# espnet/espnet

Hardware: NVIDIA H100
Metric: utterances/sec (RTF) Conformer-large ASR inference at 1/2/4/8 H100 vs CPU ref (higher is better)
Workload: dtype f32

## Files before the change

### espnet_b200/csrc/capi.cu

```cuda
#include <stdlib.h>
#include <string.h>

#include "common.cuh"
#include "gemm.h"

#ifndef ESPB_PDL_DEFAULT
#define ESPB_PDL_DEFAULT 1
#endif

static thread_local char g_err[512] = "";

void espb_set_error(const char* msg) {
  strncpy(g_err, msg ? msg : "", sizeof(g_err) - 1);
  g_err[sizeof(g_err) - 1] = 0;
}

namespace espb {
bool pdl_enabled() {
  static int v = -1;
  if (v < 0) { const char* e = getenv("ESPB_PDL"); v = e ? (e[0] == '1') : ESPB_PDL_DEFAULT; }
  return v == 1;
}
}

extern "C" {

const char* espb_last_error(void) { return g_err; }
int espb_abi_version(void) { return 7; }

int espb_device_sm(int* major, int* minor) {
  int dev = 0;
  cudaDeviceProp prop;
  if (cudaGetDevice(&dev) != cudaSuccess || cudaGetDeviceProperties(&prop, dev) != cudaSuccess) {
    espb_set_error("no CUDA device");
    return ESPB_ERR_CUDA;
  }
  *major = prop.major; *minor = prop.minor;
  return ESPB_OK;
}

int espb_gemm_f32(const EspbGemmDesc* d, int use_tc, cudaStream_t stream) {
  if (!d) { espb_set_error("gemm: null descriptor"); return ESPB_ERR_ARG; }
  if (d->a_mode < 0 || d->a_mode > 3) { espb_set_error("gemm: a_mode must be 0..3"); return ESPB_ERR_ARG; }
  return use_tc ? espb_gemm_tc_launch(*d, stream, use_tc == 2 ? 2 : 1) : espb_gemm_simt_launch(*d, stream);
}

}
```

### espnet_b200/csrc/gemm.cu

```cuda
#include <cuda.h>
#include <limits.h>

#include <algorithm>
#include <cmath>
#include <stdio.h>
#include <stdlib.h>

#include "common.cuh"
#include "gemm.h"
#include "tc_common.cuh"

namespace {

using namespace espb::tc;

constexpr int BM = 128;
constexpr int BK = 32;
constexpr int A_TILE_BYTES = BM * 128;
constexpr int NUM_THREADS = 512;
constexpr int EPI_WARP0 = 9;
constexpr int EPI_THREADS = NUM_THREADS - EPI_WARP0 * 32;
constexpr int STAGING_BYTES = 32768;
constexpr int LAUNCH_REGS = (65536 / NUM_THREADS) & ~7;
constexpr int CONSUMER_REGS = 176;
// ... 77 lines not shown
  }
#pragma unroll
  for (int i = 0; i < 4; ++i) {
    if (col + i >= N) break;
    if (e.split_out) { const float h = espb::tf32_hi(t[i]); crow[col + i] = h; crow[e.c_plane + col + i] = espb::tf32_lo(t[i], h); }
    else crow[col + i] = t[i];
  }
}

template <int BN>
__device__ __forceinline__ uint32_t staging_off(int r, int c) {
  return (uint32_t)(r * BN + ((((c >> 2) ^ ((r & 3) << 1))) << 2) + (c & 3)) * 4u;
}

template <int BN>
__device__ __forceinline__ void stage_tile(uint32_t buf, const float (&d)[BN / 2], int r0, int c0) {
#pragma unroll
  for (int j = 0; j < BN / 8; ++j)
#pragma unroll
    for (int h = 0; h < 2; ++h)
      asm volatile("st.shared.v2.f32 [%0], {%1, %2};" ::"r"(buf + staging_off<BN>(r0 + 8 * h, c0 + 8 * j)), "f"(d[4 * j + 2 * h]),
                   "f"(d[4 * j + 2 * h + 1])
                   : "memory");
}

__device__ __forceinline__ float4 ld_shared_f4(uint32_t addr) {
  float4 v;
  asm volatile("ld.shared.v4.f32 {%0, %1, %2, %3}, [%4];" : "=f"(v.x), "=f"(v.y), "=f"(v.z), "=f"(v.w) : "r"(addr) : "memory");
  return v;
}

constexpr int EPI_U = 4;

template <int BN>
__device__ __forceinline__ void epilogue_warps(const EspbGemmDesc& p, long long ntiles, int tiles_m, int tiles_n, int band, uint32_t staging,
                                               uint32_t stg_full, uint32_t stg_empty) {
  constexpr int NBUF = STAGING_BYTES / (64 * BN * 4);
  constexpr int TPR = BN / 4, RPP = EPI_THREADS / TPR;
  const int et = threadIdx.x - EPI_WARP0 * 32;
  const int r_first = et / TPR, cc = 4 * (et % TPR);
  int it = 0;
  for (long long t = blockIdx.x; t < ntiles; t += gridDim.x, ++it) {
    const TilePos tp = tile_at<BN>(p, t, tiles_m, tiles_n, band);
    EpiArgs e;
    const long long coff = (long long)tp.by * p.sc_y + (long long)tp.bx * p.sc_x;
    const long long roff = (long long)tp.by * p.sr_y + (long long)tp.bx * p.sr_x;
    e.C = p.C + coff; e.c_plane = p.c_plane; e.ldc = p.ldc; e.split_out = p.split_out;
    e.bias = p.bias ? p.bias + (long long)tp.bx * p.sbias_x : nullptr; e.R = p.R ? p.R + roff : nullptr;
    e.ldr = p.ldr; e.alpha = p.alpha; e.act = p.act;
    const bool c_vec = ((p.ldc & 3) == 0) && ((coff & 3) == 0) && ((p.c_plane & 3) == 0) && ((reinterpret_cast<uintptr_t>(p.C) & 15) == 0);
    const bool r_vec = ((p.ldr & 3) == 0) && ((reinterpret_cast<uintptr_t>(e.R) & 15) == 0);
    const int col = tp.n0 + cc;
    const float4 bv = e.bias ? ldg_quad(e.bias, col, p.N, (reinterpret_cast<uintptr_t>(e.bias) & 15) == 0) : make_float4(0.f, 0.f, 0.f, 0.f);
    for (int g = 0; g < 2; ++g) {
      mbar_wait(stg_full + 8 * g, (uint32_t)it & 1);
      const uint32_t buf = staging + (NBUF == 1 ? 0 : g) * (64 * BN * 4);
      const int row_base = tp.m0 + 64 * g;
#pragma unroll 1
      for (int r0 = r_first; r0 < 64; r0 += EPI_U * RPP) {
        float4 rv[EPI_U];
#pragma unroll
        for (int u = 0; u < EPI_U; ++u) {
          const int r = r0 + u * RPP, row = row_base + r;
          rv[u] = (e.R && r < 64 && row < p.M) ? ld_quad(e.R + (long long)row * e.ldr, col, p.N, r_vec) : make_float4(0.f, 0.f, 0.f, 0.f);
        }
#pragma unroll
        for (int u = 0; u < EPI_U; ++u) {
          const int r = r0 + u * RPP, row = row_base + r;
          if (r >= 64 || row >= p.M) break;
          const float4 a = ld_shared_f4(buf + staging_off<BN>(r, cc));
          const float v[4] = {epi_apply(e, a.x, bv.x, rv[u].x), epi_apply(e, a.y, bv.y, rv[u].y), epi_apply(e, a.z, bv.z, rv[u].z),
                              epi_apply(e, a.w, bv.w, rv[u].w)};
          epi_store4(e, row, col, v, p.N, c_vec);
        }
      }
      mbar_arrive_local(stg_empty + 8 * (NBUF == 1 ? g ^ 1 : g));
    }
  }
}

template <int BN, int STAGES, bool PROMOTE>
__global__ void __launch_bounds__(NUM_THREADS, 1)
gemm_tf32x3_kernel(const __grid_constant__ CUtensorMap tmA, const __grid_constant__ CUtensorMap tmB, EspbGemmDesc p, int bxm, int bym, int axm, int aym,
                   int tiles_m, int tiles_n, int band) {
  constexpr int B_TILE_BYTES = BN * 128;
  constexpr int STAGE_BYTES = 2 * A_TILE_BYTES + 2 * B_TILE_BYTES;
  constexpr int NR = BN / 2;
  constexpr int NBUF = STAGING_BYTES / (64 * BN * 4);
  extern __shared__ uint8_t smem_raw[];
  const uint32_t smem_base = (smem_u32(smem_raw) + 1023u) & ~1023u;
  const uint32_t staging = smem_base + STAGES * STAGE_BYTES;
  const uint32_t full_bar = staging + STAGING_BYTES, empty_bar = full_bar + 8 * STAGES;
  const uint32_t stg_full = empty_bar + 8 * STAGES, stg_empty = stg_full + 16;

  const int warp = threadIdx.x >> 5, lane = threadIdx.x & 31;
  const int num_kb = (p.K + BK - 1) / BK;
  const long long ntiles = (long long)tiles_m * tiles_n * p.nbx * p.nby;

  if (threadIdx.x == 0) {
    for (int s = 0; s < STAGES; ++s) { mbar_init(full_bar + 8 * s, 1); mbar_init(empty_bar + 8 * s, 2); }
    for (int g = 0; g < 2; ++g) { mbar_init(stg_full + 8 * g, 128); mbar_init(stg_empty + 8 * g, EPI_THREADS); }
    asm volatile("fence.mbarrier_init.release.cluster;" ::: "memory");
    asm volatile("prefetch.tensormap [%0];" ::"l"(&tmA) : "memory");
    asm volatile("prefetch.tensormap [%0];" ::"l"(&tmB) : "memory");
  }
  __syncthreads();
  espb::pdl_trigger();
  espb::pdl_wait();

  if (warp >= 8) {
    asm volatile("setmaxnreg.dec.sync.aligned.u32 %0;" ::"n"(EPI_REGS));
    if (warp >= EPI_WARP0) {
      epilogue_warps<BN>(p, ntiles, tiles_m, tiles_n, band, staging, stg_full, stg_empty);
      return;
    }
    if (elect_one_sync()) {
      const int cblk = (p.a_mode != 0) ? p.cv_cin / BK : 0;
      const ConvGeom g = conv_geom(p.a_mode);
      int s = 0;
      uint32_t ph = 0;
      for (long long t = blockIdx.x; t < ntiles; t += gridDim.x) {
        const TilePos tp = tile_at<BN>(p, t, tiles_m, tiles_n, band);
        for (int kb = 0; kb < num_kb; ++kb) {
          mbar_wait(empty_bar + 8 * s, ph ^ 1);
          const uint32_t fb = full_bar + 8 * s;
          mbar_expect_tx(fb, STAGE_BYTES);
          const uint32_t sa = smem_base + s * STAGE_BYTES;
          if (p.a_mode == 0) {
            const int ko = (p.kob > 0) ? kb / p.kob : 0;
            const int ki = (p.kob > 0) ? kb % p.kob : kb;
            tma_load_5d(sa, &tmA, fb, ki * BK, tp.m0, tp.bx * axm + ko, tp.by * aym, 0);
            tma_load_5d(sa + A_TILE_BYTES, &tmA, fb, ki * BK, tp.m0, tp.bx * axm + ko, tp.by * aym, 1);
          } else {
            const int tap = kb / cblk, c0 = (kb % cblk) * BK;
            const int kt = tap / g.k, kf = tap - kt * g.k;
            const int par = (kt % g.s) * g.s + kf % g.s;
            tma_load_5d(sa, &tmA, fb, c0, tp.m0 + kt / g.s, tp.bx + kf / g.s, par, tp.by);
            tma_load_5d(sa + A_TILE_BYTES, &tmA, fb, c0, tp.m0 + kt / g.s, tp.bx + kf / g.s, g.s * g.s + par, tp.by);
          }
          tma_load_5d(sa + 2 * A_TILE_BYTES, &tmB, fb, kb * BK, tp.n0, tp.bx * bxm, tp.by * bym, 0);
          tma_load_5d(sa + 2 * A_TILE_BYTES + B_TILE_BYTES, &tmB, fb, kb * BK, tp.n0, tp.bx * bxm, tp.by * bym, 1);
          if (++s == STAGES) { s = 0; ph ^= 1; }
        }
      }
    }
    return;
  }

  asm volatile("setmaxnreg.inc.sync.aligned.u32 %0;" ::"n"(CONSUMER_REGS));
  const int wg = warp >> 2;
  const bool wg_leader = (threadIdx.x & 127) == 0;
  const int row_in_half = (warp & 3) * 16 + (lane >> 2), col_in_tile = 2 * (lane & 3);
  const uint32_t my_buf = staging + (NBUF == 1 ? 0 : wg) * (64 * BN * 4);
  const uint32_t stg_parity0 = (NBUF == 1 && wg == 1) ? 0u : 1u;
  int s = 0;
  uint32_t ph = 0;
  float acc[NR], part[NR];
  int it = 0;
  for (long long t = blockIdx.x; t < ntiles; t += gridDim.x, ++it) {
#pragma unroll
    for (int i = 0; i < NR; ++i) { acc[i] = 0.f; part[i] = 0.f; }
    for (int kb = 0; kb < num_kb; ++kb) {
      mbar_wait(full_bar + 8 * s, ph);
      const uint32_t sa = smem_base + s * STAGE_BYTES + wg * 64 * 128;
      const uint32_t sb = smem_base + s * STAGE_BYTES + 2 * A_TILE_BYTES;
      const bool fresh = PROMOTE ? (kb % CHUNK_KB == 0) : (kb == 0);
      fence_regs(part);
      wgmma_fence();
#pragma unroll
      for (int k = 0; k < BK / 8; ++k) {
        const uint64_t a_hi = gmma_desc(sa + k * 32), a_lo = gmma_desc(sa + A_TILE_BYTES + k * 32);
        const uint64_t b_hi = gmma_desc(sb + k * 32), b_lo = gmma_desc(sb + B_TILE_BYTES + k * 32);
        wgmma_tf32<BN>(part, a_lo, b_hi, (fresh && k == 0) ? 0u : 1u);
        wgmma_tf32<BN>(part, a_hi, b_lo, 1u);
        wgmma_tf32<BN>(part, a_hi, b_hi, 1u);
      }
      wgmma_commit();
      wgmma_wait<0>();
      fence_regs(part);
      if (wg_leader) mbar_arrive_local(empty_bar + 8 * s);
      if (PROMOTE && (kb % CHUNK_KB == CHUNK_KB - 1 || kb == num_kb - 1)) {
#pragma unroll
        for (int i = 0; i < NR; ++i) acc[i] += part[i];
      }
      if (++s == STAGES) { s = 0; ph ^= 1; }
    }
    mbar_wait(stg_empty + 8 * wg, ((uint32_t)it & 1) ^ stg_parity0);
    stage_tile<BN>(my_buf, PROMOTE ? acc : part, row_in_half, col_in_tile);
    mbar_arrive_local(stg_full + 8 * wg);
  }
}

constexpr int BAND_MAX_KB = 4;
constexpr int BAND_SMEM = 232448;
constexpr int BAND_THREADS = 384;

struct BandTile {
  int k;
  int seq;
  int t, nt;
  int m0, n0;
  int bx, by;
};

__device__ __forceinline__ void band_unit(const EspbGemmDesc& p, int nmb, int k, int seq, int bn, BandTile& w) {
  const long long nunits = (long long)nmb * p.nbx * p.nby;
  for (;; ++k) {
    const long long u = blockIdx.x + (long long)k * gridDim.x;
    if (u >= nunits) { w.k = -1; return; }
    const int mb = (int)(u % nmb), z = (int)(u / nmb);
    const int m0 = mb * BM, mlast = min(p.M, m0 + BM) - 1;
    const int lo = max(0, p.band_t - 1 - mlast), hi = min(p.N - 1, 2 * p.band_t - 2 - m0);
    if (hi < lo) continue;
    const int n_start = lo & ~7;
    w.k = k; w.seq = seq; w.t = 0; w.nt = (hi - n_start) / bn + 1; w.m0 = m0; w.n0 = n_start; w.bx = z % p.nbx; w.by = z / p.nbx;
    return;
  }
}
__device__ __forceinline__ void band_next(const EspbGemmDesc& p, int nmb, int bn, BandTile& w) {
  if (w.t + 1 < w.nt) { ++w.t; w.n0 += bn; return; }
  band_unit(p, nmb, w.k + 1, w.seq + 1, bn, w);
}
// ... 222 lines not shown
      else c[0] = t;
    }
  }
}

int make_map(CUtensorMap* map, const float* base, const long long dims[5], const long long strides_el[4], int box_rows) {
  return espb_make_tensor_map(map, base, dims, strides_el, BK, box_rows, 1);
}

int num_sms() {
  static int n = 0;
  if (n == 0) {
    int dev = 0;
    cudaGetDevice(&dev);
    cudaDeviceGetAttribute(&n, cudaDevAttrMultiProcessorCount, dev);
    if (n <= 0) n = 1;
  }
  return n;
}

constexpr long long GEMM_B_L2_BYTES = 24ll << 20;
constexpr long long GEMM_B_BAND_BYTES = 8ll << 20;

int column_band(const EspbGemmDesc& d, int bn, int tiles_m, int tiles_n) {
  const double a_bytes = 2.0 * tiles_m * BM * d.K * sizeof(float), tile_b = 2.0 * bn * d.K * sizeof(float), b_bytes = tiles_n * tile_b;
  if (b_bytes <= GEMM_B_L2_BYTES) return tiles_n;
  const int w = (int)std::max(1.0, std::floor(GEMM_B_BAND_BYTES / tile_b));
  if (w >= tiles_n) return tiles_n;
  const double waves_per_b = tiles_m / std::max(1.0, (double)num_sms() / tiles_n);
  const double whole = a_bytes + b_bytes * waves_per_b, banded = a_bytes * ((tiles_n + w - 1) / w) + b_bytes;
  return banded < whole ? w : tiles_n;
}

template <int BN, int STAGES, bool PROMOTE>
int launch_tc(const CUtensorMap& tmA, const CUtensorMap& tmB, const EspbGemmDesc& d, int bxm, int bym, int axm, int aym, cudaStream_t stream) {
  constexpr int smem = STAGES * (2 * A_TILE_BYTES + 2 * BN * 128) + STAGING_BYTES + 1024 + 16 * STAGES + 32;
  static_assert(smem <= 232448, "dynamic shared memory budget exceeded");
  static bool attr_set = false;
  if (!attr_set) {
    if (cudaFuncSetAttribute(gemm_tf32x3_kernel<BN, STAGES, PROMOTE>, cudaFuncAttributeMaxDynamicSharedMemorySize, smem) != cudaSuccess) {
      espb_set_error("cudaFuncSetAttribute(max dynamic smem) failed");
      return ESPB_ERR_CUDA;
    }
    attr_set = true;
  }
  const int tiles_m = (d.M + BM - 1) / BM, tiles_n = (d.N + BN - 1) / BN;
  const int band = column_band(d, BN, tiles_m, tiles_n);
  const long long tiles = (long long)tiles_m * tiles_n * d.nbx * d.nby;
  const int grid = (int)std::min(tiles, (long long)num_sms());
  if (espb::launch_pdl(gemm_tf32x3_kernel<BN, STAGES, PROMOTE>, dim3(grid), dim3(NUM_THREADS), smem, stream, tmA, tmB, d, bxm, bym, axm, aym, tiles_m,
                       tiles_n, band) != cudaSuccess) {
    espb_set_error(cudaGetErrorString(cudaGetLastError())); return ESPB_ERR_CUDA;
  }
  return ESPB_OK;
}

void window_span(const float* base, long long ld, long long sx, long long sy, const EspbGemmDesc& d, uintptr_t& lo, uintptr_t& hi) {
  long long a = 0, b = (long long)(d.M - 1) * ld + (d.N - 1);
  const long long ex = (long long)(d.nbx - 1) * sx, ey = (long long)(d.nby - 1) * sy;
  (ex < 0 ? a : b) += ex;
  (ey < 0 ? a : b) += ey;
  lo = reinterpret_cast<uintptr_t>(base + a);
  hi = reinterpret_cast<uintptr_t>(base + b) + sizeof(float) - 1;
}

bool residual_ok(const EspbGemmDesc& d) {
  if (!d.R) return true;
  if (d.R == d.C && d.ldr == d.ldc && d.sr_x == d.sc_x && d.sr_y == d.sc_y) return true;
  uintptr_t rlo, rhi, clo, chi;
  window_span(d.R, d.ldr, d.sr_x, d.sr_y, d, rlo, rhi);
  for (int plane = 0; plane < (d.split_out ? 2 : 1); ++plane) {
    window_span(d.C + plane * d.c_plane, d.ldc, d.sc_x, d.sc_y, d, clo, chi);
    if (rlo <= chi && clo <= rhi) return false;
  }
  return true;
}

template <int NKB, bool PROMOTE>
int launch_band(const CUtensorMap& tmA, const CUtensorMap& tmB, const EspbGemmDesc& d, int bxm, int bym, int axm, int aym, cudaStream_t stream) {
  constexpr int BN = band_bn<NKB>();
  static bool attr_set = false;
  if (!attr_set) {
    if (cudaFuncSetAttribute(relpos_band_kernel<NKB, PROMOTE>, cudaFuncAttributeMaxDynamicSharedMemorySize, BAND_SMEM) != cudaSuccess) {
      espb_set_error("cudaFuncSetAttribute(max dynamic smem) failed (band GEMM)");
// ... 79 lines not shown
    if (d.kob > 0) { k_inner = (long long)d.kob * BK; n_outer = (d.K + k_inner - 1) / k_inner; }
    axm = (d.sa_x != 0 && d.nbx > 1) ? 1 : 0;
    aym = (d.sa_y != 0 && d.nby > 1) ? 1 : 0;
    long long dims[5] = {k_inner, d.M, (axm ? d.nbx : 1) + n_outer - 1, aym ? d.nby : 1, 2};
    long long str[4] = {d.lda, d.sa_x, d.sa_y, d.a_plane};
    rc = make_map(&tmA, d.A, dims, str, BM);
  } else {
    const ConvGeom g = conv_geom(d.a_mode);
    if (d.cv_cin % BK != 0 || d.K != g.k * g.k * d.cv_cin) {
      espb_set_error("conv gemm: cin must be a multiple of 32 and K = k*k*cin");
      return ESPB_ERR_ARG;
    }
    const long long sub = (long long)d.cv_f1h * d.cv_t1h * d.cv_cin, nph = g.s * g.s;
    long long dims[5] = {d.cv_cin, d.cv_t1h, d.cv_f1h, 2 * nph, d.nby};
    long long str[4] = {d.cv_cin, (long long)d.cv_t1h * d.cv_cin, sub, 2 * nph * sub};
    rc = make_map(&tmA, d.A, dims, str, BM);
  }
  if (rc != ESPB_OK) return rc;
  const int bxm = d.sb_x != 0 ? 1 : 0, bym = d.sb_y != 0 ? 1 : 0;
  if (d.band_t > 0 && d.a_mode == 0 && d.K <= BAND_MAX_KB * BK && !d.bias && !d.R && d.act == espb::ACT_NONE && !d.split_out) {
    const int nkb = (d.K + BK - 1) / BK;
    long long dims[5] = {d.K, d.N, bxm ? d.nbx : 1, bym ? d.nby : 1, 2};
    long long str[4] = {d.ldb, d.sb_x, d.sb_y, d.b_plane};
    if ((rc = make_map(&tmB, d.B, dims, str, nkb <= 3 ? band_bn<3>() : band_bn<4>())) != ESPB_OK) return rc;
    const bool pr = version == 2;
    switch (nkb) {
      case 1: return pr ? launch_band<1, true>(tmA, tmB, d, bxm, bym, axm, aym, stream) : launch_band<1, false>(tmA, tmB, d, bxm, bym, axm, aym, stream);
      case 2: return pr ? launch_band<2, true>(tmA, tmB, d, bxm, bym, axm, aym, stream) : launch_band<2, false>(tmA, tmB, d, bxm, bym, axm, aym, stream);
      case 3: return pr ? launch_band<3, true>(tmA, tmB, d, bxm, bym, axm, aym, stream) : launch_band<3, false>(tmA, tmB, d, bxm, bym, axm, aym, stream);
      default: return pr ? launch_band<4, true>(tmA, tmB, d, bxm, bym, axm, aym, stream) : launch_band<4, false>(tmA, tmB, d, bxm, bym, axm, aym, stream);
    }
  }
  const long long tiles_m = (d.M + BM - 1) / BM, nb = (long long)d.nbx * d.nby;
  const int bn = (d.N <= 64 || tiles_m * ((d.N + 127) / 128) * nb < num_sms()) ? 64 : 128;
  {
    long long dims[5] = {d.K, d.N, bxm ? d.nbx : 1, bym ? d.nby : 1, 2};
    long long str[4] = {d.ldb, d.sb_x, d.sb_y, d.b_plane};
    rc = make_map(&tmB, d.B, dims, str, bn);
    if (rc != ESPB_OK) return rc;
  }
  if (version == 2) {
    if (bn == 128) return launch_tc<128, 3, true>(tmA, tmB, d, bxm, bym, axm, aym, stream);
    return launch_tc<64, 4, true>(tmA, tmB, d, bxm, bym, axm, aym, stream);
  }
  if (bn == 128) return launch_tc<128, 3, false>(tmA, tmB, d, bxm, bym, axm, aym, stream);
  return launch_tc<64, 4, false>(tmA, tmB, d, bxm, bym, axm, aym, stream);
}

int espb_gemm_simt_launch(const EspbGemmDesc& d, cudaStream_t stream) {
  if (d.M <= 0 || d.N <= 0 || d.K <= 0 || d.nbx <= 0 || d.nby <= 0) { espb_set_error("gemm: bad shape"); return ESPB_ERR_ARG; }
  if (!residual_ok(d)) { espb_set_error("gemm: residual R partially overlaps the output C"); return ESPB_ERR_ARG; }
  dim3 grid((d.M + 63) / 64, (d.N + 63) / 64, d.nbx * d.nby);
  gemm_simt_kernel<<<grid, 256, 0, stream>>>(d);
  ESPB_CHECK_LAUNCH();
  return ESPB_OK;
}
```

### espnet_b200/csrc/gemm.h

```cpp
#pragma once
#include <cuda_runtime.h>

struct EspbGemmDesc {
  int M, N, K;
  int nbx, nby;
  int a_mode;
  int kob;
  const float* A; long long a_plane, lda, sa_x, sa_y;
  const float* B; long long b_plane, ldb, sb_x, sb_y;
  float* C; long long c_plane, ldc, sc_x, sc_y;
  int split_out;
  const float* bias;
  long long sbias_x;
  const float* R; long long ldr, sr_x, sr_y;
  float alpha;
  int act;
  int cv_t1h, cv_f1h, cv_cin;
  int band_t;
};

struct ConvGeom { int k, s; };
__host__ __device__ __forceinline__ ConvGeom conv_geom(int a_mode) {
  return a_mode == 2 ? ConvGeom{3, 1} : a_mode == 3 ? ConvGeom{5, 3} : ConvGeom{3, 2};
}

int espb_gemm_tc_launch(const EspbGemmDesc& d, cudaStream_t stream, int version);
int espb_gemm_simt_launch(const EspbGemmDesc& d, cudaStream_t stream);
```

### espnet_b200/lib.py

```python
import ctypes
import os
from ctypes import POINTER, Structure, c_float, c_int, c_longlong, c_void_p

import torch

_HERE = os.path.dirname(os.path.abspath(__file__))
LIB_PATH = os.path.join(_HERE, "libespnet_b200.so")

_lib = None


class GemmDesc(Structure):

    _fields_ = [
        ("M", c_int), ("N", c_int), ("K", c_int), ("nbx", c_int), ("nby", c_int), ("a_mode", c_int), ("kob", c_int),
        ("A", c_void_p), ("a_plane", c_longlong), ("lda", c_longlong), ("sa_x", c_longlong), ("sa_y", c_longlong),
        ("B", c_void_p), ("b_plane", c_longlong), ("ldb", c_longlong), ("sb_x", c_longlong), ("sb_y", c_longlong),
        ("C", c_void_p), ("c_plane", c_longlong), ("ldc", c_longlong), ("sc_x", c_longlong), ("sc_y", c_longlong),
        ("split_out", c_int), ("bias", c_void_p), ("sbias_x", c_longlong),
        ("R", c_void_p), ("ldr", c_longlong), ("sr_x", c_longlong), ("sr_y", c_longlong),
        ("alpha", c_float), ("act", c_int), ("cv_t1h", c_int), ("cv_f1h", c_int), ("cv_cin", c_int), ("band_t", c_int),
    ]


P, I, L, F = c_void_p, c_int, c_longlong, c_float

_SIGS = {
    "espb_gemm_f32": [POINTER(GemmDesc), I, P],
    "espb_stft_logmel_f32": [P, P, I, I, I, P, P, P, P, P, P, P, I, I, P, I, P, P],
    "espb_utt_mvn_from_partial_f32": [P, P, I, I, I, I, P, P],
    "espb_utt_mvn_f32": [P, P, I, I, I, P, P],
    "espb_global_mvn_f32": [P, P, I, I, I, P, P, I, I, P],
    "espb_layernorm_f32": [P, L, I, P, P, F, P, P, L, P],
    "espb_split_tf32_f32": [P, L, P, L, P],
    "espb_conv1_relu_f32": [P, I, I, I, P, P, I, P, I, I, I, I, P],
    "espb_conv1_relu_phase_f32": [P, I, I, I, P, P, I, P, I, I, I, I, I, P],
    "espb_phase_split_f32": [P, L, I, I, I, I, I, I, I, P, P],
    "espb_qu_qv_f32": [P, L, L, I, P, P, P, P, L, P],
    "espb_v_transpose_f32": [P, L, I, I, I, I, P, P, L, I, P],
    "espb_relpos_softmax_f32": [P, P, I, I, I, I, I, P, F, P, L, P],
    "espb_masked_softmax_f32": [P, I, I, I, I, P, F, P, L, P],
    "espb_flash_attn_f32": [P, L, L, L, P, L, L, L, P, L, I, P, I, P, I, I, I, I, P, L, L, P],
    "espb_glu_dwconv_bn_swish_f32": [P, I, I, I, P, P, P, I, P, P, P, L, P],
    "espb_zero_pad_rows_f32": [P, I, I, I, P, L, I, P],
    "espb_csgu_f32": [P, I, I, I, P, P, P, F, P, P, I, P, P, L, P],
    "espb_merge_dwconv_f32": [P, I, I, I, P, P, P, I, P, L, P],
    "espb_branch_pool_f32": [P, P, L, I, I, I, P, P, P, P, P, P, P, P],
    "espb_branch_merge_f32": [P, P, L, L, I, I, P, F, F, P, L, P],
    "espb_cbe_build_chunks_f32": [P, I, I, I, I, I, I, P, I, I, F, P, P, P, P],
    "espb_cbe_ctx_propagate_f32": [P, I, I, I, I, P, P, I, I, P],
    "espb_zero_rows_f32": [P, L, L, L, I, L, I, P],
    "espb_gather_rows_f32": [P, I, L, P, I, I, P, P],
    "espb_log_softmax_rows_f32": [P, L, L, I, P],
    "espb_argmax_rows_f32": [P, L, L, I, P, P],
# ... 90 lines not shown
```

### espnet_b200/ops.py

```python
import os

import torch

from . import lib
from .lib import GemmDesc, call, ptr

ACT_NONE, ACT_RELU, ACT_SWISH, ACT_GELU = 0, 1, 2, 3

_GEMM_MODE = os.environ.get("ESPNET_B200_GEMM", "tc2")
launch_counter = [0]
gemm_profile = None


def set_gemm_mode(mode):
    global _GEMM_MODE
    assert mode in ("tc", "tc2", "simt")
    _GEMM_MODE = mode


def gemm_mode():
    return _GEMM_MODE


def _count(n=1):
    launch_counter[0] += n


def new_split(*shape, device="cuda"):
    return torch.empty((2,) + tuple(shape), dtype=torch.float32, device=device)


def split_from(x):
    x = x.contiguous()
    out = new_split(*x.shape, device=x.device)
    call("espb_split_tf32_f32", ptr(x), x.numel(), ptr(out), x.numel())
    _count()
    return out


def gemm(M, N, K, A, a_plane, lda, B, b_plane, ldb, C, ldc, *, c_plane=0, split_out=False, bias=None, R=None, ldr=0,
         alpha=1.0, act=ACT_NONE, nbx=1, nby=1, sa=(0, 0), sb=(0, 0), sc=(0, 0), sr=(0, 0), kob=0, a_mode=0, conv=(0, 0, 0),
         a_off=0, b_off=0, c_off=0, r_off=0, sbias_x=0, bias_off=0, band_t=0, force=None):
    d = GemmDesc()
    d.M, d.N, d.K, d.nbx, d.nby, d.a_mode, d.kob = M, N, K, nbx, nby, a_mode, kob
    d.A = A.data_ptr() + 4 * a_off
    d.a_plane, d.lda, d.sa_x, d.sa_y = a_plane, lda, sa[0], sa[1]
    d.B = B.data_ptr() + 4 * b_off
    d.b_plane, d.ldb, d.sb_x, d.sb_y = b_plane, ldb, sb[0], sb[1]
    d.C = C.data_ptr() + 4 * c_off
    d.c_plane, d.ldc, d.sc_x, d.sc_y = c_plane, ldc, sc[0], sc[1]
    d.split_out = 1 if split_out else 0
    d.bias = (bias.data_ptr() + 4 * bias_off) if bias is not None else None
    d.sbias_x = sbias_x
    d.R = (R.data_ptr() + 4 * r_off) if R is not None else None
    d.ldr, d.sr_x, d.sr_y = ldr, sr[0], sr[1]
    d.alpha, d.act = float(alpha), act
    d.cv_t1h, d.cv_f1h, d.cv_cin = conv
    d.band_t = band_t
    mode = force or _GEMM_MODE
    use_tc = {"tc": 1, "tc2": 2}.get(mode, 0)
    if use_tc:
        al = [lda, ldb, a_plane, b_plane, sa[0], sa[1], sb[0], sb[1], a_off, b_off]
        if any(v % 4 for v in al):
            use_tc = 0
        if a_mode and conv[2] % 32:
            use_tc = 0
        if a_mode == 0 and kob > 0 and K % (kob * 32):
            use_tc = 0
    if lib.profile is not None:
        lib.profile_tag[0] = f"{'tc' + str(use_tc) if use_tc else 'simt'} M{M} N{N} K{K} x{nbx * nby}" + (" conv" if a_mode else "")
    prof = gemm_profile if use_tc else None
    if prof is not None:
        e0, e1 = torch.cuda.Event(enable_timing=True), torch.cuda.Event(enable_timing=True)
        e0.record()
    call("espb_gemm_f32", d, use_tc)
    if prof is not None:
        e1.record()
        n_alg = band_t if band_t > 0 else N
        prof.append((2.0 * M * n_alg * K * nbx * nby, e0, e1))
    _count()
    return bool(use_tc)


def linear(x_split, w_split, out, *, bias=None, act=ACT_NONE, residual=None, alpha=1.0, split_out=False, force=None):
    M, K = x_split.shape[1], x_split.shape[2]
    N = w_split.shape[1]
    assert w_split.shape[2] == K
    return gemm(M, N, K, x_split, M * K, K, w_split, N * K, K, out, N, c_plane=M * N, split_out=split_out, bias=bias,
                R=residual, ldr=N, alpha=alpha, act=act, force=force)


_ATTN_MODE = os.environ.get("ESPB_ATTN", "fused")


def set_attn_mode(mode):
    global _ATTN_MODE
    assert mode in ("fused", "materialized")
    _ATTN_MODE = mode


def attn_mode():
    return _ATTN_MODE


def use_flash_attn(dk):
    return _ATTN_MODE == "fused" and dk == 64 and _GEMM_MODE != "simt"


def flash_attn(q_split, q_off, ldq, k_split, k_off, ldk, vt, Tp, bd, Rp, lens32, B, H, T, dk, out_split):
    call("espb_flash_attn_f32", ptr(q_split), q_off, q_split[0].numel(), ldq, ptr(k_split), k_off, k_split[0].numel(), ldk, ptr(vt),
         vt[0].numel(), Tp, ptr(bd), Rp, ptr(lens32), B, H, T, dk, ptr(out_split), out_split[0].numel(), H * dk)
    _count()


def layernorm(x, gamma, beta, eps, out_plain=None, out_split=None):
    rows, D = x.numel() // x.shape[-1], x.shape[-1]
    plane = out_split[0].numel() if out_split is not None else 0
    call("espb_layernorm_f32", ptr(x), rows, D, ptr(gamma), ptr(beta), eps, ptr(out_plain), ptr(out_split), plane)
    _count()


def log_softmax_rows_(x2d):
# ... 13 lines not shown
```

### include/espnet_b200.h

```cpp
#ifndef ESPNET_B200_H
#define ESPNET_B200_H

#include <cuda_runtime.h>

#ifdef __cplusplus
extern "C" {
#endif

#define ESPB_ACT_NONE 0
#define ESPB_ACT_RELU 1
#define ESPB_ACT_SWISH 2
#define ESPB_ACT_GELU 3

const char* espb_last_error(void);
int espb_abi_version(void);
int espb_device_sm(int* major, int* minor);

typedef struct EspbGemmDesc {
  int M, N, K;
  int nbx, nby;
  int a_mode;
  int kob;
  const float* A; long long a_plane, lda, sa_x, sa_y;
  const float* B; long long b_plane, ldb, sb_x, sb_y;
  float* C; long long c_plane, ldc, sc_x, sc_y;
  int split_out;
  const float* bias; long long sbias_x;
  const float* R; long long ldr, sr_x, sr_y;
  float alpha;
  int act;
  int cv_t1h, cv_f1h, cv_cin;
  int band_t;
} EspbGemmDesc;
int espb_gemm_f32(const EspbGemmDesc* d, int use_tc, cudaStream_t stream);

int espb_frontend_blocks(int Tf_max);
int espb_stft_logmel_f32(const float* wave, const long long* wave_lens, int B, int Lmax, int hop, const float* window, const float* tw512,
                         const float* tw256t, const int* mel_start, const int* mel_count, const int* mel_offset, const float* mel_weight,
                         int mel_nnz, int n_mels, float* out, int Tf_max, float* partial, cudaStream_t stream);
int espb_utt_mvn_from_partial_f32(float* feats, const long long* wave_lens, int B, int Tf_max, int n_mels, int hop, const float* partial,
                                  cudaStream_t stream);
int espb_utt_mvn_f32(float* feats, const long long* feat_lens, int B, int Tf_max, int n_mels, float* partial_ws, cudaStream_t stream);
int espb_global_mvn_f32(float* feats, const long long* feat_lens, int B, int Tmax, int D, const float* mean, const float* stdv, int norm_means,
                        int norm_vars, cudaStream_t stream);

int espb_layernorm_f32(const float* x, long long rows, int D, const float* gamma, const float* beta, float eps, float* out_plain,
                       float* out_split, long long split_plane, cudaStream_t stream);
int espb_split_tf32_f32(const float* x, long long n, float* out, long long plane, cudaStream_t stream);
int espb_conv1_relu_f32(const float* feats, int B, int Tf_max, int F, const float* w, const float* bias, int C, float* out, int T1, int F1,
                        int T1h, int F1h, cudaStream_t stream);
int espb_conv1_relu_phase_f32(const float* feats, int B, int Tf_max, int F, const float* w, const float* bias, int C, float* out, int T1, int F1,
                              int s, int T1h, int F1h, cudaStream_t stream);
int espb_phase_split_f32(const float* x, long long x_plane, int B, int F, int T, int C, int s, int Th, int Fh, float* out, cudaStream_t stream);
int espb_qu_qv_f32(const float* qkv, long long qkv_plane, long long M, int D, const float* pos_u, const float* pos_v, float* qu, float* qv,
                   long long out_plane, cudaStream_t stream);
int espb_v_transpose_f32(const float* qkv, long long qkv_plane, int B, int Tmax, int D, int H, const int* lens, float* vt,
                         long long vt_plane, int Tp, cudaStream_t stream);
int espb_relpos_softmax_f32(const float* ac, const float* bd, int B, int H, int T, int Tp, int Rp, const int* lens, float sqrt_dk,
                            float* probs, long long probs_plane, cudaStream_t stream);
int espb_masked_softmax_f32(const float* scores, int B, int H, int T, int Tp, const int* lens, float sqrt_dk, float* probs, long long probs_plane,
                            cudaStream_t stream);
int espb_flash_attn_f32(const float* q, long long q_off, long long q_plane, long long ldq, const float* k, long long k_off, long long k_plane,
                        long long ldk, const float* vt, long long vt_plane, int Tp, const float* bd, int Rp, const int* lens, int B, int H, int T,
                        int dk, float* out, long long out_plane, long long ldo, cudaStream_t stream);
int espb_glu_dwconv_bn_swish_f32(const float* y, int B, int Tmax, int C, const int* lens, const float* dw_w, const float* dw_b, int K,
// ... 68 lines not shown
```

Before: 182.4.

## Add split-K stream-K style path to TF32x3 TMA GEMM with workspace reduction

Adds optional split-K for the promoted TF32x3 tensor-core GEMM when a caller supplies a workspace. Each tile is divided into K-chunk units spread across CTAs. Non-leading splits stage partial chunk sums to global slots, and the last arriving unit reduces them with atomic tickets before applying the epilogue. A host cost model picks the split factor and BN to fill the SMs for small-tile-count GEMMs, at the price of extra global traffic and synchronisation.

```diff
diff --git a/espnet_b200/csrc/capi.cu b/espnet_b200/csrc/capi.cu
--- a/espnet_b200/csrc/capi.cu
+++ b/espnet_b200/csrc/capi.cu
@@ -42,6 +42,10 @@
 int espb_gemm_f32(const EspbGemmDesc* d, int use_tc, cudaStream_t stream) {
   if (!d) { espb_set_error("gemm: null descriptor"); return ESPB_ERR_ARG; }
   if (d->a_mode < 0 || d->a_mode > 3) { espb_set_error("gemm: a_mode must be 0..3"); return ESPB_ERR_ARG; }
+  if (d->ws && ((reinterpret_cast<uintptr_t>(d->ws) & 15) || d->ws_bytes < 0)) {
+    espb_set_error("gemm: split-K workspace must be 16-byte aligned with ws_bytes >= 0");
+    return ESPB_ERR_ARG;
+  }
   return use_tc ? espb_gemm_tc_launch(*d, stream, use_tc == 2 ? 2 : 1) : espb_gemm_simt_launch(*d, stream);
 }
 
diff --git a/espnet_b200/csrc/gemm.cu b/espnet_b200/csrc/gemm.cu
--- a/espnet_b200/csrc/gemm.cu
+++ b/espnet_b200/csrc/gemm.cu
@@ -133,6 +133,59 @@
 
 constexpr int EPI_U = 4;
 
+struct SplitK {
+  int S;
+  int cpu;
+  int nch;
+  int nslots;
+  float* part;
+  int* ctr;
+};
+
+__device__ __forceinline__ float4 ld_cg_f4(const float* ptr) {
+  float4 v;
+  asm volatile("ld.global.cg.v4.f32 {%0, %1, %2, %3}, [%4];" : "=f"(v.x), "=f"(v.y), "=f"(v.z), "=f"(v.w) : "l"(ptr) : "memory");
+  return v;
+}
+__device__ __forceinline__ void add_f4(float4& a, const float4& b) { a.x += b.x; a.y += b.y; a.z += b.z; a.w += b.w; }
+__device__ __forceinline__ void epi_bar_sync() { asm volatile("bar.sync 1, %0;" ::"n"(EPI_THREADS) : "memory"); }
+
+template <int BN>
+__device__ __forceinline__ void stage_to_slot(int rows, float* slot, uint32_t staging, uint32_t stg_full, uint32_t stg_empty, int it,
+                                              int r_first, int cc) {
+  constexpr int NBUF = STAGING_BYTES / (64 * BN * 4);
+  constexpr int RPP = EPI_THREADS / (BN / 4);
+  for (int g = 0; g < 2; ++g) {
+    mbar_wait(stg_full + 8 * g, (uint32_t)it & 1);
+    const uint32_t buf = staging + (NBUF == 1 ? 0 : g) * (64 * BN * 4);
+#pragma unroll 1
+    for (int r = r_first; r < min(64, rows - 64 * g); r += RPP)
+      *reinterpret_cast<float4*>(slot + (64 * g + r) * BN + cc) = ld_shared_f4(buf + staging_off<BN>(r, cc));
+    mbar_arrive_local(stg_empty + 8 * (NBUF == 1 ? g ^ 1 : g));
+  }
+}
+
+struct TileEpi {
+  EpiArgs e;
+  bool c_vec, r_vec;
+  int col;
+  float4 bv;
+};
+__device__ __forceinline__ TileEpi tile_epi(const EspbGemmDesc& p, const TilePos& tp, int cc) {
+  TileEpi te;
+  EpiArgs& e = te.e;
+  const long long coff = (long long)tp.by * p.sc_y + (long long)tp.bx * p.sc_x;
+  const long long roff = (long long)tp.by * p.sr_y + (long long)tp.bx * p.sr_x;
+  e.C = p.C + coff; e.c_plane = p.c_plane; e.ldc = p.ldc; e.split_out = p.split_out;
+  e.bias = p.bias ? p.bias + (long long)tp.bx * p.sbias_x : nullptr; e.R = p.R ? p.R + roff : nullptr;
+  e.ldr = p.ldr; e.alpha = p.alpha; e.act = p.act;
+  te.c_vec = ((p.ldc & 3) == 0) && ((coff & 3) == 0) && ((p.c_plane & 3) == 0) && ((reinterpret_cast<uintptr_t>(p.C) & 15) == 0);
+  te.r_vec = ((p.ldr & 3) == 0) && ((reinterpret_cast<uintptr_t>(e.R) & 15) == 0);
+  te.col = tp.n0 + cc;
+  te.bv = e.bias ? ldg_quad(e.bias, te.col, p.N, (reinterpret_cast<uintptr_t>(e.bias) & 15) == 0) : make_float4(0.f, 0.f, 0.f, 0.f);
+  return te;
+}
+
 template <int BN>
 __device__ __forceinline__ void epilogue_warps(const EspbGemmDesc& p, long long ntiles, int tiles_m, int tiles_n, int band, uint32_t staging,
                                                uint32_t stg_full, uint32_t stg_empty) {
@@ -143,16 +196,8 @@
   int it = 0;
   for (long long t = blockIdx.x; t < ntiles; t += gridDim.x, ++it) {
     const TilePos tp = tile_at<BN>(p, t, tiles_m, tiles_n, band);
-    EpiArgs e;
-    const long long coff = (long long)tp.by * p.sc_y + (long long)tp.bx * p.sc_x;
-    const long long roff = (long long)tp.by * p.sr_y + (long long)tp.bx * p.sr_x;
-    e.C = p.C + coff; e.c_plane = p.c_plane; e.ldc = p.ldc; e.split_out = p.split_out;
-    e.bias = p.bias ? p.bias + (long long)tp.bx * p.sbias_x : nullptr; e.R = p.R ? p.R + roff : nullptr;
-    e.ldr = p.ldr; e.alpha = p.alpha; e.act = p.act;
-    const bool c_vec = ((p.ldc & 3) == 0) && ((coff & 3) == 0) && ((p.c_plane & 3) == 0) && ((reinterpret_cast<uintptr_t>(p.C) & 15) == 0);
-    const bool r_vec = ((p.ldr & 3) == 0) && ((reinterpret_cast<uintptr_t>(e.R) & 15) == 0);
-    const int col = tp.n0 + cc;
-    const float4 bv = e.bias ? ldg_quad(e.bias, col, p.N, (reinterpret_cast<uintptr_t>(e.bias) & 15) == 0) : make_float4(0.f, 0.f, 0.f, 0.f);
+    const TileEpi te = tile_epi(p, tp, cc);
+    const EpiArgs& e = te.e;
     for (int g = 0; g < 2; ++g) {
       mbar_wait(stg_full + 8 * g, (uint32_t)it & 1);
       const uint32_t buf = staging + (NBUF == 1 ? 0 : g) * (64 * BN * 4);
@@ -163,16 +208,16 @@
 #pragma unroll
         for (int u = 0; u < EPI_U; ++u) {
           const int r = r0 + u * RPP, row = row_base + r;
-          rv[u] = (e.R && r < 64 && row < p.M) ? ld_quad(e.R + (long long)row * e.ldr, col, p.N, r_vec) : make_float4(0.f, 0.f, 0.f, 0.f);
+          rv[u] = (e.R && r < 64 && row < p.M) ? ld_quad(e.R + (long long)row * e.ldr, te.col, p.N, te.r_vec) : make_float4(0.f, 0.f, 0.f, 0.f);
         }
 #pragma unroll
         for (int u = 0; u < EPI_U; ++u) {
           const int r = r0 + u * RPP, row = row_base + r;
           if (r >= 64 || row >= p.M) break;
           const float4 a = ld_shared_f4(buf + staging_off<BN>(r, cc));
-          const float v[4] = {epi_apply(e, a.x, bv.x, rv[u].x), epi_apply(e, a.y, bv.y, rv[u].y), epi_apply(e, a.z, bv.z, rv[u].z),
-                              epi_apply(e, a.w, bv.w, rv[u].w)};
-          epi_store4(e, row, col, v, p.N, c_vec);
+          const float v[4] = {epi_apply(e, a.x, te.bv.x, rv[u].x), epi_apply(e, a.y, te.bv.y, rv[u].y), epi_apply(e, a.z, te.bv.z, rv[u].z),
+                              epi_apply(e, a.w, te.bv.w, rv[u].w)};
+          epi_store4(e, row, te.col, v, p.N, te.c_vec);
         }
       }
       mbar_arrive_local(stg_empty + 8 * (NBUF == 1 ? g ^ 1 : g));
@@ -180,10 +225,56 @@
   }
 }
 
+template <int BN>
+__device__ __forceinline__ void epilogue_split_warps(const EspbGemmDesc& p, long long ntiles, int tiles_m, int tiles_n, int band,
+                                                     uint32_t staging, uint32_t stg_full, uint32_t stg_empty, const SplitK& sk, int* ticket) {
+  constexpr int TPR = BN / 4, RPP = EPI_THREADS / TPR;
+  constexpr int SLOT = BM * BN;
+  const int et = threadIdx.x - EPI_WARP0 * 32;
+  const int r_first = et / TPR, cc = 4 * (et % TPR);
+  int it = 0;
+  const long long nunits = ntiles * sk.S;
+  for (long long u = blockIdx.x; u < nunits; u += gridDim.x) {
+    const long long t = u / sk.S;
+    const int sp = (int)(u - t * sk.S);
+    const TilePos tp = tile_at<BN>(p, t, tiles_m, tiles_n, band);
+    float* const tws = sk.part + t * sk.nslots * SLOT;
+    const int c0 = sp * sk.cpu, c1 = min(c0 + sk.cpu, sk.nch);
+    for (int c = sp == 0 ? c1 - 1 : c0; c < c1; ++c, ++it)
+      stage_to_slot<BN>(p.M - tp.m0, tws + (sp == 0 ? 0 : 1 + c - sk.cpu) * SLOT, staging, stg_full, stg_empty, it, r_first, cc);
+    __threadfence();
+    epi_bar_sync();
+    if (et == 0) *ticket = atomicAdd(sk.ctr + t, 1);
+    epi_bar_sync();
+    if (*reinterpret_cast<volatile int*>(ticket) != sk.S - 1) continue;
+    __threadfence();
+    const TileEpi te = tile_epi(p, tp, cc);
+    const EpiArgs& e = te.e;
+    for (int r = r_first; r < BM; r += RPP) {
+      const int row = tp.m0 + r;
+      if (row >= p.M) break;
+      const float* const src = tws + r * BN + cc;
+      const float4 rv = e.R ? ld_quad(e.R + (long long)row * e.ldr, te.col, p.N, te.r_vec) : make_float4(0.f, 0.f, 0.f, 0.f);
+      float4 a = ld_cg_f4(src);
+      int k = 1;
+      for (; k + 4 <= sk.nslots; k += 4) {
+        const float4 v0 = ld_cg_f4(src + k * SLOT), v1 = ld_cg_f4(src + (k + 1) * SLOT), v2 = ld_cg_f4(src + (k + 2) * SLOT),
+                     v3 = ld_cg_f4(src + (k + 3) * SLOT);
+        add_f4(a, v0); add_f4(a, v1); add_f4(a, v2); add_f4(a, v3);
+      }
+      for (; k < sk.nslots; ++k) add_f4(a, ld_cg_f4(src + k * SLOT));
+      const float v[4] = {epi_apply(e, a.x, te.bv.x, rv.x), epi_apply(e, a.y, te.bv.y, rv.y), epi_apply(e, a.z, te.bv.z, rv.z),
+                          epi_apply(e, a.w, te.bv.w, rv.w)};
+      epi_store4(e, row, te.col, v, p.N, te.c_vec);
+    }
+    if (et == 0) sk.ctr[t] = 0;
+  }
+}
+
 template <int BN, int STAGES, bool PROMOTE>
 __global__ void __launch_bounds__(NUM_THREADS, 1)
 gemm_tf32x3_kernel(const __grid_constant__ CUtensorMap tmA, const __grid_constant__ CUtensorMap tmB, EspbGemmDesc p, int bxm, int bym, int axm, int aym,
-                   int tiles_m, int tiles_n, int band) {
+                   int tiles_m, int tiles_n, int band, SplitK sk) {
   constexpr int B_TILE_BYTES = BN * 128;
   constexpr int STAGE_BYTES = 2 * A_TILE_BYTES + 2 * B_TILE_BYTES;
   constexpr int NR = BN / 2;
@@ -197,6 +288,9 @@
   const int warp = threadIdx.x >> 5, lane = threadIdx.x & 31;
   const int num_kb = (p.K + BK - 1) / BK;
   const long long ntiles = (long long)tiles_m * tiles_n * p.nbx * p.nby;
+  const long long nunits = ntiles * sk.S;
+  const int kb_split = sk.S > 1 ? sk.cpu * CHUNK_KB : num_kb;
+  __shared__ int split_ticket;
 
   if (threadIdx.x == 0) {
     for (int s = 0; s < STAGES; ++s) { mbar_init(full_bar + 8 * s, 1); mbar_init(empty_bar + 8 * s, 2); }
@@ -212,7 +306,8 @@
   if (warp >= 8) {
     asm volatile("setmaxnreg.dec.sync.aligned.u32 %0;" ::"n"(EPI_REGS));
     if (warp >= EPI_WARP0) {
-      epilogue_warps<BN>(p, ntiles, tiles_m, tiles_n, band, staging, stg_full, stg_empty);
+      if (PROMOTE && sk.S > 1) epilogue_split_warps<BN>(p, ntiles, tiles_m, tiles_n, band, staging, stg_full, stg_empty, sk, &split_ticket);
+      else epilogue_warps<BN>(p, ntiles, tiles_m, tiles_n, band, staging, stg_full, stg_empty);
       return;
     }
     if (elect_one_sync()) {
@@ -220,9 +315,11 @@
       const ConvGeom g = conv_geom(p.a_mode);
       int s = 0;
       uint32_t ph = 0;
-      for (long long t = blockIdx.x; t < ntiles; t += gridDim.x) {
+      for (long long u = blockIdx.x; u < nunits; u += gridDim.x) {
+        const long long t = u / sk.S;
         const TilePos tp = tile_at<BN>(p, t, tiles_m, tiles_n, band);
-        for (int kb = 0; kb < num_kb; ++kb) {
+        const int kb0 = (int)(u - t * sk.S) * kb_split, kb1 = min(kb0 + kb_split, num_kb);
+        for (int kb = kb0; kb < kb1; ++kb) {
           mbar_wait(empty_bar + 8 * s, ph ^ 1);
           const uint32_t fb = full_bar + 8 * s;
           mbar_expect_tx(fb, STAGE_BYTES);
@@ -258,10 +355,19 @@
   uint32_t ph = 0;
   float acc[NR], part[NR];
   int it = 0;
-  for (long long t = blockIdx.x; t < ntiles; t += gridDim.x, ++it) {
+  auto handover = [&](const float (&v)[NR]) {
+    mbar_wait(stg_empty + 8 * wg, ((uint32_t)it & 1) ^ stg_parity0);
+    stage_tile<BN>(my_buf, v, row_in_half, col_in_tile);
+    mbar_arrive_local(stg_full + 8 * wg);
+    ++it;
+  };
+  for (long long u = blockIdx.x; u < nunits; u += gridDim.x) {
+    const long long t = u / sk.S;
+    const int sp = (int)(u - t * sk.S);
+    const int kb0 = sp * kb_split, kb1 = min(kb0 + kb_split, num_kb);
 #pragma unroll
     for (int i = 0; i < NR; ++i) { acc[i] = 0.f; part[i] = 0.f; }
-    for (int kb = 0; kb < num_kb; ++kb) {
+    for (int kb = kb0; kb < kb1; ++kb) {
       mbar_wait(full_bar + 8 * s, ph);
       const uint32_t sa = smem_base + s * STAGE_BYTES + wg * 64 * 128;
       const uint32_t sb = smem_base + s * STAGE_BYTES + 2 * A_TILE_BYTES;
@@ -281,14 +387,16 @@
       fence_regs(part);
       if (wg_leader) mbar_arrive_local(empty_bar + 8 * s);
       if (PROMOTE && (kb % CHUNK_KB == CHUNK_KB - 1 || kb == num_kb - 1)) {
-#pragma unroll
-        for (int i = 0; i < NR; ++i) acc[i] += part[i];
+        if (sp == 0) {
+#pragma unroll
+          for (int i = 0; i < NR; ++i) acc[i] += part[i];
+        } else {
+          handover(part);
+        }
       }
       if (++s == STAGES) { s = 0; ph ^= 1; }
     }
-    mbar_wait(stg_empty + 8 * wg, ((uint32_t)it & 1) ^ stg_parity0);
-    stage_tile<BN>(my_buf, PROMOTE ? acc : part, row_in_half, col_in_tile);
-    mbar_arrive_local(stg_full + 8 * wg);
+    if (sp == 0) handover(PROMOTE ? acc : part);
   }
 }
 
@@ -577,8 +685,49 @@
   return banded < whole ? w : tiles_n;
 }
 
+constexpr long long SPLIT_CTR_BYTES = 4096;
+constexpr double SPLIT_SLOT_COST = 0.25;
+constexpr double SPLIT_MIN_GAIN = 0.9;
+constexpr int SPLIT_MAX_WAVES = 2;
+
+long long split_ws_need(long long tiles, int nslots, int bn) { return SPLIT_CTR_BYTES + tiles * nslots * BM * bn * (long long)sizeof(float); }
+
+int choose_split(const EspbGemmDesc& d, int bn0, SplitK& sk) {
+  const int sms = num_sms();
+  const long long tiles_m = (d.M + BM - 1) / BM, nb = (long long)d.nbx * d.nby;
+  const int nch = ((d.K + BK - 1) / BK + CHUNK_KB - 1) / CHUNK_KB;
+  if (nch < 2 || tiles_m * ((d.N + 63) / 64) * nb > (long long)SPLIT_MAX_WAVES * sms) return bn0;
+  auto cost = [&](int bn, int cpu, int S, int nslots) {
+    const long long units = tiles_m * ((d.N + bn - 1) / bn) * nb * S;
+    const double c = (double)((units + sms - 1) / sms) * cpu + (S > 1 ? SPLIT_SLOT_COST * (cpu + nslots) : 0.0);
+    return c * bn / 64;
+  };
+  const double base = cost(bn0, nch, 1, 0);
+  double best = SPLIT_MIN_GAIN * base;
+  int best_bn = bn0;
+  for (int bn = 64; bn <= (d.N > 64 ? 128 : 64); bn += 64) {
+    const long long tiles = tiles_m * ((d.N + bn - 1) / bn) * nb;
+    if (tiles > SPLIT_CTR_BYTES / (long long)sizeof(int)) continue;
+    for (int cpu = nch - 1; cpu >= 1; --cpu) {
+      const int S = (nch + cpu - 1) / cpu, nslots = 1 + nch - cpu;
+      if (split_ws_need(tiles, nslots, bn) > d.ws_bytes) continue;
+      const double c = cost(bn, cpu, S, nslots);
+      if (c < best) {
+        best = c; best_bn = bn;
+        sk.S = S; sk.cpu = cpu; sk.nch = nch; sk.nslots = nslots;
+      }
+    }
+  }
+  if (sk.S > 1) {
+    sk.ctr = reinterpret_cast<int*>(d.ws);
+    sk.part = d.ws + SPLIT_CTR_BYTES / sizeof(float);
+  }
+  return best_bn;
+}
+
 template <int BN, int STAGES, bool PROMOTE>
-int launch_tc(const CUtensorMap& tmA, const CUtensorMap& tmB, const EspbGemmDesc& d, int bxm, int bym, int axm, int aym, cudaStream_t stream) {
+int launch_tc(const CUtensorMap& tmA, const CUtensorMap& tmB, const EspbGemmDesc& d, int bxm, int bym, int axm, int aym, const SplitK& sk,
+              cudaStream_t stream) {
   constexpr int smem = STAGES * (2 * A_TILE_BYTES + 2 * BN * 128) + STAGING_BYTES + 1024 + 16 * STAGES + 32;
   static_assert(smem <= 232448, "dynamic shared memory budget exceeded");
   static bool attr_set = false;
@@ -591,10 +740,10 @@
   }
   const int tiles_m = (d.M + BM - 1) / BM, tiles_n = (d.N + BN - 1) / BN;
   const int band = column_band(d, BN, tiles_m, tiles_n);
-  const long long tiles = (long long)tiles_m * tiles_n * d.nbx * d.nby;
-  const int grid = (int)std::min(tiles, (long long)num_sms());
+  const long long units = (long long)tiles_m * tiles_n * d.nbx * d.nby * sk.S;
+  const int grid = (int)std::min(units, (long long)num_sms());
   if (espb::launch_pdl(gemm_tf32x3_kernel<BN, STAGES, PROMOTE>, dim3(grid), dim3(NUM_THREADS), smem, stream, tmA, tmB, d, bxm, bym, axm, aym, tiles_m,
-                       tiles_n, band) != cudaSuccess) {
+                       tiles_n, band, sk) != cudaSuccess) {
     espb_set_error(cudaGetErrorString(cudaGetLastError())); return ESPB_ERR_CUDA;
   }
   return ESPB_OK;
@@ -740,7 +889,9 @@
     }
   }
   const long long tiles_m = (d.M + BM - 1) / BM, nb = (long long)d.nbx * d.nby;
-  const int bn = (d.N <= 64 || tiles_m * ((d.N + 127) / 128) * nb < num_sms()) ? 64 : 128;
+  int bn = (d.N <= 64 || tiles_m * ((d.N + 127) / 128) * nb < num_sms()) ? 64 : 128;
+  SplitK sk{1, 0, 0, 0, nullptr, nullptr};
+  if (version == 2 && d.a_mode == 0 && d.ws) bn = choose_split(d, bn, sk);
   {
     long long dims[5] = {d.K, d.N, bxm ? d.nbx : 1, bym ? d.nby : 1, 2};
     long long str[4] = {d.ldb, d.sb_x, d.sb_y, d.b_plane};
@@ -748,11 +899,11 @@
     if (rc != ESPB_OK) return rc;
   }
   if (version == 2) {
-    if (bn == 128) return launch_tc<128, 3, true>(tmA, tmB, d, bxm, bym, axm, aym, stream);
-    return launch_tc<64, 4, true>(tmA, tmB, d, bxm, bym, axm, aym, stream);
-  }
-  if (bn == 128) return launch_tc<128, 3, false>(tmA, tmB, d, bxm, bym, axm, aym, stream);
-  return launch_tc<64, 4, false>(tmA, tmB, d, bxm, bym, axm, aym, stream);
+    if (bn == 128) return launch_tc<128, 3, true>(tmA, tmB, d, bxm, bym, axm, aym, sk, stream);
+    return launch_tc<64, 4, true>(tmA, tmB, d, bxm, bym, axm, aym, sk, stream);
+  }
+  if (bn == 128) return launch_tc<128, 3, false>(tmA, tmB, d, bxm, bym, axm, aym, sk, stream);
+  return launch_tc<64, 4, false>(tmA, tmB, d, bxm, bym, axm, aym, sk, stream);
 }
 
 int espb_gemm_simt_launch(const EspbGemmDesc& d, cudaStream_t stream) {
diff --git a/espnet_b200/csrc/gemm.h b/espnet_b200/csrc/gemm.h
--- a/espnet_b200/csrc/gemm.h
+++ b/espnet_b200/csrc/gemm.h
@@ -17,6 +17,8 @@
   int act;
   int cv_t1h, cv_f1h, cv_cin;
   int band_t;
+  float* ws;
+  long long ws_bytes;
 };
 
 struct ConvGeom { int k, s; };
diff --git a/espnet_b200/lib.py b/espnet_b200/lib.py
--- a/espnet_b200/lib.py
+++ b/espnet_b200/lib.py
@@ -20,6 +20,7 @@
         ("split_out", c_int), ("bias", c_void_p), ("sbias_x", c_longlong),
         ("R", c_void_p), ("ldr", c_longlong), ("sr_x", c_longlong), ("sr_y", c_longlong),
         ("alpha", c_float), ("act", c_int), ("cv_t1h", c_int), ("cv_f1h", c_int), ("cv_cin", c_int), ("band_t", c_int),
+        ("ws", c_void_p), ("ws_bytes", c_longlong),
     ]
 
 
diff --git a/espnet_b200/ops.py b/espnet_b200/ops.py
--- a/espnet_b200/ops.py
+++ b/espnet_b200/ops.py
@@ -40,7 +40,7 @@
 
 def gemm(M, N, K, A, a_plane, lda, B, b_plane, ldb, C, ldc, *, c_plane=0, split_out=False, bias=None, R=None, ldr=0,
          alpha=1.0, act=ACT_NONE, nbx=1, nby=1, sa=(0, 0), sb=(0, 0), sc=(0, 0), sr=(0, 0), kob=0, a_mode=0, conv=(0, 0, 0),
-         a_off=0, b_off=0, c_off=0, r_off=0, sbias_x=0, bias_off=0, band_t=0, force=None):
+         a_off=0, b_off=0, c_off=0, r_off=0, sbias_x=0, bias_off=0, band_t=0, ws=None, force=None):
     d = GemmDesc()
     d.M, d.N, d.K, d.nbx, d.nby, d.a_mode, d.kob = M, N, K, nbx, nby, a_mode, kob
     d.A = A.data_ptr() + 4 * a_off
@@ -57,6 +57,8 @@
     d.alpha, d.act = float(alpha), act
     d.cv_t1h, d.cv_f1h, d.cv_cin = conv
     d.band_t = band_t
+    if ws is not None:
+        d.ws, d.ws_bytes = ws.data_ptr(), ws.numel() * ws.element_size()
     mode = force or _GEMM_MODE
     use_tc = {"tc": 1, "tc2": 2}.get(mode, 0)
     if use_tc:
@@ -82,12 +84,13 @@
     return bool(use_tc)
 
 
-def linear(x_split, w_split, out, *, bias=None, act=ACT_NONE, residual=None, alpha=1.0, split_out=False, force=None):
+def linear(x_split, w_split, out, *, bias=None, act=ACT_NONE, residual=None, alpha=1.0, split_out=False, ws=None, force=None):
     M, K = x_split.shape[1], x_split.shape[2]
     N = w_split.shape[1]
     assert w_split.shape[2] == K
+    extra = {} if ws is None else {"ws": ws}
     return gemm(M, N, K, x_split, M * K, K, w_split, N * K, K, out, N, c_plane=M * N, split_out=split_out, bias=bias,
-                R=residual, ldr=N, alpha=alpha, act=act, force=force)
+                R=residual, ldr=N, alpha=alpha, act=act, force=force, **extra)
 
 
 _ATTN_MODE = os.environ.get("ESPB_ATTN", "fused")
diff --git a/include/espnet_b200.h b/include/espnet_b200.h
--- a/include/espnet_b200.h
+++ b/include/espnet_b200.h
@@ -31,6 +31,8 @@
   int act;
   int cv_t1h, cv_f1h, cv_cin;
   int band_t;
+  float* ws;
+  long long ws_bytes;
 } EspbGemmDesc;
 int espb_gemm_f32(const EspbGemmDesc* d, int use_tc, cudaStream_t stream);
 
```

Result: slower. 179.3, median of 6 (-1.7%).
